# google/vizier

Hardware: NVIDIA H100
Metric: GP-UCB candidates scored/sec (higher is better)
Workload: dtype f64

## Files before the change

vizier_b200/csrc/async.cuh:

```cuda
#pragma once
#include <cuda.h>
#include <stdint.h>

namespace vzgp {

__device__ __forceinline__ void cp_async16(void* smem_dst, const void* gsrc, bool valid) {
  const unsigned s = static_cast<unsigned>(__cvta_generic_to_shared(smem_dst));
  const int sz = valid ? 16 : 0;
  asm volatile("cp.async.cg.shared.global [%0], [%1], 16, %2;\n" ::"r"(s), "l"(gsrc), "r"(sz) : "memory");
}
__device__ __forceinline__ void cp_async_commit() { asm volatile("cp.async.commit_group;\n" ::: "memory"); }
template <int N>
__device__ __forceinline__ void cp_async_wait() {
  asm volatile("cp.async.wait_group %0;\n" ::"n"(N) : "memory");
}
__device__ __forceinline__ unsigned smem_u32(const void* p) { return static_cast<unsigned>(__cvta_generic_to_shared(p)); }
__device__ __forceinline__ void mbar_init(uint64_t* bar, unsigned count) {
  asm volatile("mbarrier.init.shared::cta.b64 [%0], %1;\n" ::"r"(smem_u32(bar)), "r"(count) : "memory");
}
__device__ __forceinline__ void mbar_expect_tx(uint64_t* bar, unsigned bytes) {
  asm volatile("mbarrier.arrive.expect_tx.shared::cta.b64 _, [%0], %1;\n" ::"r"(smem_u32(bar)), "r"(bytes) : "memory");
}
__device__ __forceinline__ void mbar_wait(uint64_t* bar, unsigned parity) {
  unsigned ok;
  do {
    asm volatile(
        "{\n.reg .pred p;\nmbarrier.try_wait.parity.shared::cta.b64 p, [%1], %2;\nselp.u32 %0, 1, 0, p;\n}\n"
        : "=r"(ok)
        : "r"(smem_u32(bar)), "r"(parity)
        : "memory");
  } while (!ok);
}
__device__ __forceinline__ void tma_load_2d(void* smem_dst, const CUtensorMap* map, int c0, int c1, uint64_t* bar) {
  asm volatile(
      "cp.async.bulk.tensor.2d.shared::cluster.global.mbarrier::complete_tx::bytes [%0], [%1, {%2, %3}], [%4];\n" ::"r"(smem_u32(smem_dst)),
      "l"(reinterpret_cast<uint64_t>(map)), "r"(c0), "r"(c1), "r"(smem_u32(bar))
      : "memory");
}
__device__ __forceinline__ void fence_proxy_async() { asm volatile("fence.proxy.async;\n" ::: "memory"); }

__device__ __forceinline__ unsigned cluster_ctarank() {
  unsigned r;
  asm volatile("mov.u32 %0, %%cluster_ctarank;\n" : "=r"(r));
  return r;
}
__device__ __forceinline__ unsigned cluster_nctarank() {
  unsigned r;
  asm volatile("mov.u32 %0, %%cluster_nctarank;\n" : "=r"(r));
  return r;
}
__device__ __forceinline__ void cluster_sync() {
  asm volatile("barrier.cluster.arrive.release;\nbarrier.cluster.wait.acquire;\n" ::: "memory");
}
__device__ __forceinline__ void mbar_arrive_cluster(const uint64_t* bar, unsigned rank) {
  asm volatile(
      "{\n.reg .b32 ra;\nmapa.shared::cluster.u32 ra, %0, %1;\nmbarrier.arrive.shared::cluster.b64 _, [ra];\n}\n" ::"r"(
          smem_u32(bar)),
      "r"(rank)
      : "memory");
}
__device__ __forceinline__ void tma_load_2d_multicast(void* smem_dst, const CUtensorMap* map, int c0, int c1, uint64_t* bar,
                                                      uint16_t cta_mask) {
  asm volatile(
      "cp.async.bulk.tensor.2d.shared::cluster.global.mbarrier::complete_tx::bytes.multicast::cluster [%0], [%1, {%2, %3}], [%4], %5;\n" ::"r"(
          smem_u32(smem_dst)),
      "l"(reinterpret_cast<uint64_t>(map)), "r"(c0), "r"(c1), "r"(smem_u32(bar)), "h"(cta_mask)
      : "memory");
}


}
```

vizier_b200/csrc/score.cu:

```cuda
#include <cuda.h>

#include <climits>
#include <cstring>
#include <map>
#include <mutex>
#include <tuple>

#include "launchers.h"
#include "matern_fast.cuh"
#include "score_small.cuh"
#include "topk_merge.cuh"
#include "tiles.cuh"

namespace vzgp {

using GP1 = GemmCfg<64, 64, 16, 4, 4>;
constexpr int kThreads = 256;
constexpr int kBlockThreads = 288;
static_assert(GP1::kThreads == kThreads, "phase 1 maps one d2 block to every math thread");

constexpr int kBN = 128;
constexpr int kBK = 32;
constexpr int kStages = 4;
__host__ __device__ constexpr int pair_pos(int r) { return (((r >> 4) * 8 + (r & 7)) << 1) | ((r >> 3) & 1); }
__host__ __device__ constexpr int pair_row(int pos) { return ((pos >> 4) << 4) + ((pos >> 1) & 7) + ((pos & 1) << 3); }
static_assert(pair_row(pair_pos(13)) == 13 && pair_row(pair_pos(58)) == 58 && pair_pos(8) == 1, "pair order round trip");
constexpr int kABox = (kTM / 2) * 16;
constexpr int kBHalf = kBN * 16;
constexpr int kStageDoubles = 4 * kABox + 2 * kBHalf;
constexpr unsigned kStageBytes = kStageDoubles * sizeof(double);
constexpr int kCluster = 2;
constexpr int kBPieces = kCluster < 2 ? 2 : kCluster;
constexpr int kBPieceRows = 2 * kBN / kBPieces;
static_assert(kBPieces % 2 == 0 && kBN % (kBPieces / 2) == 0, "B pieces tile the two halves of a stage");

#ifdef VZ_SCORE_TIMING
constexpr int kScoreCounters = 11;
__device__ unsigned long long g_score_t[kScoreCounters];
#define VZ_ST(...) __VA_ARGS__
#else
#define VZ_ST(...)
#endif

template <bool WITH_LINF, bool GENERIC>
__global__ void __launch_bounds__(kBlockThreads, 1) k_score(const __grid_constant__ ScoreArgs a) {
  extern __shared__ double smem_raw[];
  double* smem = smem_raw + (((1024u - (static_cast<unsigned>(__cvta_generic_to_shared(smem_raw)) & 1023u)) & 1023u) >> 3);
  constexpr int LD = kLD1;
  const int dc = a.kp.dc, dk = a.kp.dk, np = a.np;
  double* ring = smem;
  double* sa = ring;
  double* sb = sa + dc * LD;
  double* s_alpha = ring + (kStages * kStageDoubles > 3 * kMaxDc * kLD1 ? kStages * kStageDoubles : 3 * kMaxDc * kLD1);
  double* s_mu = s_alpha + 128;
  double* s_linf = s_mu + 64;
  double* s_rowsq = s_linf + 64;
  uint64_t* full_bar = reinterpret_cast<uint64_t*>(s_rowsq + 256);
  uint64_t* empty_bar = full_bar + kStages;
  int32_t* za = reinterpret_cast<int32_t*>(full_bar + 8);
  int32_t* zb = za + dk * LD;
  uint8_t* s_mask = reinterpret_cast<uint8_t*>(zb + dk * LD);

  const int tid = threadIdx.x, lane = tid & 31, warp = tid >> 5;
  const int ty = tid / 16, tx = tid % 16;
  const int wm = warp & 1, wn = warp >> 1;
  const int fr = lane >> 2, fk = lane & 3;
  const int pr = ((fr & 1) << 2) | (fr >> 1);
  double* scr = a.scratch + (size_t)blockIdx.x * kTM * np;
  const unsigned crank = cluster_ctarank(), ncta = cluster_nctarank();
  auto tile_gate = [&]() { if (ncta > 1) cluster_sync(); else __syncthreads(); };
  if (tid < kMaxDc) s_mask[tid] = a.tr.mask[tid];
  if (tid == 0) {
    for (int s = 0; s < kStages; ++s) { mbar_init(full_bar + s, 1); mbar_init(empty_bar + s, ncta * (kThreads / 32)); }
    asm volatile("fence.mbarrier_init.release.cluster;\n" ::: "memory");
  }
  tile_gate();
  int clamped = 0;
  unsigned slab_n = 0;
  const bool is_producer = warp == kThreads / 32;
  auto consumer_sync = [&]() { asm volatile("bar.sync 1, %0;\n" ::"n"(kThreads) : "memory"); };
  VZ_ST(long long t_p1 = 0, t_gate = 0, t_p2 = 0, t_tile = 0, t_wait = 0, w_tile = 0, n_tiles = 0;)
  VZ_ST(long long t_d2 = 0, t_mat = 0, t_st = 0, t_sync = 0;)

  const int ntiles = (a.M + kTM - 1) / kTM;
  const int nblocks = (np + kBN - 1) / kBN;
  const int nsplit = a.nsplit;
  const double* XTs = a.XT;
  const double* XTu = a.XT + (size_t)dc * np;

  for (int w0 = blockIdx.x - crank; w0 < ntiles * nsplit; w0 += gridDim.x) {
    const int work = w0 + crank;
    const int tile = work / nsplit, split = work - tile * nsplit;
    const int m0 = tile * kTM;
    const int nq = (nsplit == 1) ? nblocks : ((split == nblocks - 1 - split) ? 1 : 2);
    auto block_of = [&](int q) { return (nsplit == 1) ? q : (q == 0 ? split : nblocks - 1 - split); };
    auto slabs_in = [&](int jb) { int kend = (jb + 1) * kBN; if (kend > np) kend = np; return kend / kBK; };
    if (is_producer) {
      tile_gate();
      VZ_ST(w_tile = 0;)
      if (lane == 0) {
        const uint16_t cmask = (uint16_t)((1u << ncta) - 1u);
        for (int q = 0; q < nq; ++q) {
          const int jb = block_of(q), nsl = slabs_in(jb);
          for (int ks = 0; ks < nsl; ++ks) {
            const int stage = slab_n % kStages;
            VZ_ST(const long long t0 = clock64();)
            mbar_wait(empty_bar + stage, ((slab_n / kStages) & 1) ^ 1);
            VZ_ST(w_tile += clock64() - t0;)
            double* base = ring + stage * kStageDoubles;
            const int k0 = ks * kBK;
            mbar_expect_tx(full_bar + stage, kStageBytes);
            for (int h = 0; h < 4; ++h)
              tma_load_2d(base + h * kABox, &a.mapA, 2 * k0 + 16 * h, (int)blockIdx.x * (kTM / 2), full_bar + stage);
            for (int p = (int)crank; p < kBPieces; p += (int)ncta) {
              const int half = p / (kBPieces / 2), r0 = (p % (kBPieces / 2)) * kBPieceRows;
              double* dst = base + 4 * kABox + half * kBHalf + r0 * 16;
              if (ncta > 1) tma_load_2d_multicast(dst, &a.mapB, k0 + 16 * half, jb * kBN + r0, full_bar + stage, cmask);
              else tma_load_2d(dst, &a.mapB, k0 + 16 * half, jb * kBN + r0, full_bar + stage);
            }
            ++slab_n;
          }
        }
      }
      __syncwarp();
      VZ_ST(if (m0 < a.M) t_wait += w_tile;)
      continue;
    }
    VZ_ST(const long long t_tile0 = clock64(); w_tile = 0;)
    consumer_sync();
    for (int e = tid; e < kTM * dc; e += kThreads) {
      const int r = e / dc, d = e - r * dc;
      const int gr = m0 + r;
      const double v = gr < a.M ? __ldg(a.Xs + (size_t)gr * dc + d) : 0.0;
      sa[d * LD + pair_pos(r)] = WITH_LINF ? v : v * a.kp.inv_ls_c[d];
    }
    if (dk > 0) stage_rows_T_i32(a.Zs, a.M, dk, m0, kTM, za, LD, kThreads);

    auto stage_trials = [&](int jb, int buf) {
      double* dst = sb + buf * dc * LD;
      const double* src = WITH_LINF ? XTu : XTs;
      for (int c = tid; c < dc * 32; c += kThreads) {
        const int d = c >> 5, q = c & 31;
        cp_async16(dst + d * LD + q * 2, src + (size_t)d * np + jb * 64 + q * 2, true);
      }
      if (tid < 32) cp_async16(s_alpha + buf * 64 + tid * 2, a.alpha + jb * 64 + tid * 2, true);
    };
    double mu_part[4], lmin[4];
#pragma unroll
    for (int i = 0; i < 4; ++i) { mu_part[i] = 0.0; lmin[i] = INFINITY; }
    const int nj = np / 64;
    stage_trials(0, 0);
    cp_async_commit();
    for (int jb = 0; jb < nj; ++jb) {
      VZ_ST(long long tc = clock64();)
      const int buf = jb & 1;
      if (jb + 1 < nj) stage_trials(jb + 1, buf ^ 1);
      cp_async_commit();
      cp_async_wait<1>();
      consumer_sync();
      if (dk > 0) {
        stage_rows_T_i32(a.Z, np, dk, jb * 64, 64, zb, LD, kThreads);
        consumer_sync();
      }
      VZ_ST(t_sync += clock64() - tc; tc = clock64();)
      const double* sbj = sb + buf * dc * LD;
      const double* alj = s_alpha + buf * 64;
      double d2[4][4], lf[4][4];
#pragma unroll
      for (int i = 0; i < 4; ++i)
#pragma unroll
        for (int j = 0; j < 4; ++j) { d2[i][j] = 0.0; lf[i][j] = 0.0; }
      for (int d = 0; d < dc; ++d) {
        const double2 a0 = *reinterpret_cast<const double2*>(sa + d * LD + GP1::row_of(ty, 0));
        const double2 a1 = *reinterpret_cast<const double2*>(sa + d * LD + GP1::row_of(ty, 2));
        const double2 b0 = *reinterpret_cast<const double2*>(sbj + d * LD + GP1::col_of(tx, 0));
        const double2 b1 = *reinterpret_cast<const double2*>(sbj + d * LD + GP1::col_of(tx, 2));
        const double aa[4] = {a0.x, a0.y, a1.x, a1.y}, bb[4] = {b0.x, b0.y, b1.x, b1.y};
        if (WITH_LINF) {
          const double w = a.kp.inv_ls2_c[d];
          const bool in_tr = s_mask[d] != 0;
#pragma unroll
          for (int i = 0; i < 4; ++i)
#pragma unroll
            for (int j = 0; j < 4; ++j) {
              const double df = aa[i] - bb[j];
              d2[i][j] = fma(df * df, w, d2[i][j]);
              if (in_tr) lf[i][j] = fmax(lf[i][j], fabs(df));
            }
        } else {
#pragma unroll
          for (int i = 0; i < 4; ++i)
#pragma unroll
            for (int j = 0; j < 4; ++j) {
              const double df = aa[i] - bb[j];
              d2[i][j] = fma(df, df, d2[i][j]);
            }
        }
      }
      for (int k = 0; k < dk; ++k) {
        const double w = a.kp.inv_ls2_k[k];
#pragma unroll
        for (int i = 0; i < 4; ++i) {
          const int avz = za[k * LD + pair_row(GP1::row_of(ty, i))];
#pragma unroll
          for (int j = 0; j < 4; ++j) d2[i][j] += (avz != zb[k * LD + GP1::col_of(tx, j)]) ? w : 0.0;
        }
      }
      VZ_ST(t_d2 += clock64() - tc; tc = clock64();)
      if (WITH_LINF) {
#pragma unroll
        for (int i = 0; i < 4; ++i)
#pragma unroll
          for (int j = 0; j < 4; ++j)
            if ((jb * 64 + GP1::col_of(tx, j)) < a.tr.rows) lmin[i] = fmin(lmin[i], lf[i][j]);
      }
      double kv[4][4];
#pragma unroll
      for (int i = 0; i < 4; ++i)
#pragma unroll
        for (int j = 0; j < 4; ++j) kv[i][j] = matern52_fast(d2[i][j], a.kp.sf2);
#pragma unroll
      for (int i = 0; i < 4; ++i)
#pragma unroll
        for (int j = 0; j < 4; ++j) {
          const int cj = GP1::col_of(tx, j);
          kv[i][j] = (jb * 64 + cj) < a.n_valid ? kv[i][j] : 0.0;
          mu_part[i] = fma(kv[i][j], alj[cj], mu_part[i]);
        }
      VZ_ST(t_mat += clock64() - tc; tc = clock64();)
#pragma unroll
      for (int ip = 0; ip < 2; ++ip) {
        double* dst = scr + (size_t)(GP1::row_of(ty, 2 * ip) >> 1) * (2 * np) + 2 * jb * 64;
#pragma unroll
        for (int j = 0; j < 4; ++j)
          *reinterpret_cast<double2*>(dst + 2 * GP1::col_of(tx, j)) = make_double2(kv[2 * ip][j], kv[2 * ip + 1][j]);
      }
      VZ_ST(t_st += clock64() - tc;)
      VZ_ST(tc = clock64();)
      consumer_sync();
      VZ_ST(t_sync += clock64() - tc;)
    }
    cp_async_wait<0>();
#pragma unroll
    for (int i = 0; i < 4; ++i) {
#pragma unroll
      for (int o = 8; o > 0; o >>= 1) {
        mu_part[i] += __shfl_xor_sync(0xffffffffu, mu_part[i], o);
        if (WITH_LINF) lmin[i] = fmin(lmin[i], __shfl_xor_sync(0xffffffffu, lmin[i], o));
      }
      if (tx == 0) {
        s_mu[pair_row(GP1::row_of(ty, i))] = mu_part[i];
        s_linf[pair_row(GP1::row_of(ty, i))] = lmin[i];
      }
    }
    fence_proxy_async();
    VZ_ST(const long long t1 = clock64();)
    tile_gate();
    VZ_ST(const long long t2 = clock64();)

    double rowsq[2][2] = {{0.0, 0.0}, {0.0, 0.0}};
    for (int q = 0; q < nq; ++q) {
      const int jb = block_of(q);
      double acc[2][2][4][2];
#pragma unroll
      for (int mf = 0; mf < 2; ++mf)
#pragma unroll
        for (int f = 0; f < 2; ++f)
#pragma unroll
          for (int g = 0; g < 4; ++g) { acc[mf][f][g][0] = 0.0; acc[mf][f][g][1] = 0.0; }
      const int nsl = slabs_in(jb);
      const int col_base = jb * kBN + wn * 32;
      for (int ks = 0; ks < nsl; ++ks) {
        const int stage = slab_n % kStages;
        VZ_ST(const long long tw = clock64();)
        mbar_wait(full_bar + stage, (slab_n / kStages) & 1);
        VZ_ST(w_tile += clock64() - tw;)
        ++slab_n;
        const double* stg = ring + stage * kStageDoubles;
        const double* Arow0 = stg + (wm * 16 + fr) * 16;
        const double* Brow0 = stg + 4 * kABox + (wn * 32 + pr) * 16;
        const int k0 = ks * kBK;
        auto group = [&](int h, bool diag) {
          const int co = ((((h & 1) * 4 + fk) ^ pr) * 2);
          auto live = [&](int g) { return !(diag && g < h); };
          double2 b[4];
#pragma unroll
          for (int g = 0; g < 4; ++g)
            if (live(g)) b[g] = *reinterpret_cast<const double2*>(Brow0 + (h >> 1) * kBHalf + g * 8 * 16 + co);
#pragma unroll
          for (int mf = 0; mf < 2; ++mf) {
            const double* Ah = Arow0 + h * kABox + mf * 8 * 16;
            const double2 a01 = *reinterpret_cast<const double2*>(Ah + (((2 * fk) ^ fr) * 2));
            const double2 a23 = *reinterpret_cast<const double2*>(Ah + (((2 * fk + 1) ^ fr) * 2));
#pragma unroll
            for (int g = 0; g < 4; ++g)
              if (live(g))
                dmma_16x8x8(acc[mf][0][g][0], acc[mf][0][g][1], acc[mf][1][g][0], acc[mf][1][g][1],
                            a01.x, a01.y, a23.x, a23.y, b[g].x, b[g].y);
          }
        };
        if (k0 < col_base) {
#pragma unroll 1
          for (int h = 0; h < 4; ++h) group(h, false);
        } else if (k0 == col_base) {
#pragma unroll 1
          for (int h = 0; h < 4; ++h) group(h, true);
        }
        __syncwarp();
        if ((unsigned)lane < ncta) mbar_arrive_cluster(empty_bar + stage, lane);
      }
#pragma unroll
      for (int mf = 0; mf < 2; ++mf)
#pragma unroll
        for (int f = 0; f < 2; ++f)
#pragma unroll
          for (int g = 0; g < 4; ++g) {
            rowsq[mf][f] = fma(acc[mf][f][g][0], acc[mf][f][g][0], rowsq[mf][f]);
            rowsq[mf][f] = fma(acc[mf][f][g][1], acc[mf][f][g][1], rowsq[mf][f]);
          }
    }
    VZ_ST(const long long t3 = clock64();)
    cp_async_wait<0>();
#pragma unroll
    for (int mf = 0; mf < 2; ++mf)
#pragma unroll
      for (int f = 0; f < 2; ++f) {
        rowsq[mf][f] += __shfl_xor_sync(0xffffffffu, rowsq[mf][f], 1);
        rowsq[mf][f] += __shfl_xor_sync(0xffffffffu, rowsq[mf][f], 2);
        if (fk == 0) s_rowsq[wn * 64 + wm * 32 + mf * 16 + f * 8 + fr] = rowsq[mf][f];
      }
    consumer_sync();
    if (tid < kTM) {
      const int r = tid, m = m0 + r;
      if (m < a.M) {
        const double rs = (s_rowsq[r] + s_rowsq[64 + r]) + (s_rowsq[128 + r] + s_rowsq[192 + r]);
        if (nsplit == 1) {
          emit_score<GENERIC>(a, m, rs, s_mu[r], s_linf[r], clamped);
        } else {
          a.part[(size_t)split * a.mpad + m] = rs;
          if (split == 0) {
            a.part[(size_t)nsplit * a.mpad + m] = s_mu[r];
            a.part[(size_t)(nsplit + 1) * a.mpad + m] = s_linf[r];
          }
        }
      }
    }
    VZ_ST(if (m0 < a.M) { t_p1 += t1 - t_tile0; t_gate += t2 - t1; t_p2 += t3 - t2; t_tile += clock64() - t_tile0; t_wait += w_tile; ++n_tiles; })
  }
  if (clamped) atomicAdd(a.clamp_count, clamped);
#ifdef VZ_SCORE_TIMING
  if (lane == 0) {
    if (is_producer) {
      atomicAdd(&g_score_t[6], (unsigned long long)t_wait);
    } else {
      atomicAdd(&g_score_t[5], (unsigned long long)t_wait);
      if (warp == 0) {
        atomicAdd(&g_score_t[0], (unsigned long long)n_tiles);
        atomicAdd(&g_score_t[1], (unsigned long long)t_p1);
        atomicAdd(&g_score_t[2], (unsigned long long)t_p2);
        atomicAdd(&g_score_t[3], (unsigned long long)t_gate);
        atomicAdd(&g_score_t[4], (unsigned long long)t_tile);
        atomicAdd(&g_score_t[7], (unsigned long long)t_d2);
        atomicAdd(&g_score_t[8], (unsigned long long)t_mat);
        atomicAdd(&g_score_t[9], (unsigned long long)t_st);
        atomicAdd(&g_score_t[10], (unsigned long long)t_sync);
      }
    }
  }
#endif
  if (ncta > 1) cluster_sync();
}

__global__ void k_score_finalize(const ScoreArgs a) {
  const int m = blockIdx.x * blockDim.x + threadIdx.x;
  int clamped = 0;
  if (m < a.M) {
    double rs = 0.0;
    for (int s = 0; s < a.nsplit; ++s) rs += a.part[(size_t)s * a.mpad + m];
    emit_score(a, m, rs, a.part[(size_t)a.nsplit * a.mpad + m], a.part[(size_t)(a.nsplit + 1) * a.mpad + m], clamped);
  }
  if (clamped) atomicAdd(a.clamp_count, clamped);
}

template <bool WITH_LINF>
__global__ void __launch_bounds__(kSmallThreads) k_cross_small(const ScoreArgs a) {
  extern __shared__ double smem_raw[];
  cross_small_block<WITH_LINF>(a, blockIdx.x, blockIdx.y >> 2, blockIdx.y & 3, smem_raw);
}
__global__ void __launch_bounds__(kSmallThreads) k_var_small(const __grid_constant__ ScoreArgs a) {
  extern __shared__ double smem_raw[];
  var_small_dispatch(a, blockIdx.x, blockIdx.y, smem_raw);
}
template <bool WITH_LINF>
__global__ void __launch_bounds__(256) k_small_finalize(const ScoreArgs a) {
  const int m = blockIdx.x * 32 + (threadIdx.x >> 3);
  int clamped = 0;
  small_finalize_8<WITH_LINF>(a, m, threadIdx.x & 7, m < a.M, clamped);
  if (clamped) atomicAdd(a.clamp_count, clamped);
}

size_t cross_small_smem_bytes(int dc, int dk) { return sizeof(double) * 2 * dc * kLD1 + sizeof(int32_t) * 2 * dk * kLD1; }
size_t var_small_smem_bytes() {
  const size_t cp = sizeof(double) * kVarStages * kVarStageDoubles, tma = 1024 + sizeof(double) * kVarStages * kVarTmaStageDoubles;
  return cp > tma ? cp : tma;
}

typedef CUresult (*EncodeTiledFn)(CUtensorMap*, CUtensorMapDataType, cuuint32_t, void*, const cuuint64_t*,
                                  const cuuint64_t*, const cuuint32_t*, const cuuint32_t*, CUtensorMapInterleave,
                                  CUtensorMapSwizzle, CUtensorMapL2promotion, CUtensorMapFloatOOBfill);

static EncodeTiledFn encode_tiled_fn() {
  static const EncodeTiledFn fn = [] {
    void* p = nullptr;
    cudaDriverEntryPointQueryResult qres;
    EncodeTiledFn f = nullptr;
    if (cudaGetDriverEntryPoint("cuTensorMapEncodeTiled", &p, cudaEnableDefault, &qres) == cudaSuccess &&
        qres == cudaDriverEntryPointSuccess)
      f = reinterpret_cast<EncodeTiledFn>(p);
    cudaGetLastError();
    return f;
  }();
  return fn;
}

static int make_map(CUtensorMap* m, const double* base, uint64_t rows, uint64_t cols, uint64_t ld, uint32_t box_rows,
                    bool l2_promotion = true) {
  EncodeTiledFn fn = encode_tiled_fn();
  if (!fn) { set_error("cuTensorMapEncodeTiled is not available from this driver"); return VZGP_ERR_CUDA; }
  cuuint64_t gdim[2] = {cols, rows};
  cuuint64_t gstride[1] = {ld * sizeof(double)};
  cuuint32_t box[2] = {16, box_rows};
  cuuint32_t estr[2] = {1, 1};
  CUresult r = fn(m, CU_TENSOR_MAP_DATA_TYPE_FLOAT64, 2, const_cast<double*>(base), gdim, gstride, box, estr,
                  CU_TENSOR_MAP_INTERLEAVE_NONE, CU_TENSOR_MAP_SWIZZLE_128B,
                  l2_promotion ? CU_TENSOR_MAP_L2_PROMOTION_L2_256B : CU_TENSOR_MAP_L2_PROMOTION_NONE,
                  CU_TENSOR_MAP_FLOAT_OOB_FILL_NONE);
  if (r != CUDA_SUCCESS) { set_error("cuTensorMapEncodeTiled failed with CUresult %d", (int)r); return VZGP_ERR_CUDA; }
  return 0;
}

int make_tensor_map_f64(void* map, const double* base, uint64_t rows, uint64_t cols, uint64_t ld, uint32_t box_rows) {
  static const bool promo = [] { const char* e = getenv("VZGP_DF_L2PROMO"); return e && e[0] == '1'; }();
  return make_map(static_cast<CUtensorMap*>(map), base, rows, cols, ld, box_rows, promo);
}

int make_tensor_map_u8(void* map, const void* base, int rank, const uint64_t* dims, const uint64_t* strides,
                       const uint32_t* box, bool promote_256) {
  EncodeTiledFn fn = encode_tiled_fn();
  if (!fn) { set_error("cuTensorMapEncodeTiled is not available from this driver"); return VZGP_ERR_CUDA; }
  cuuint64_t gdim[3], gstride[2];
  cuuint32_t bx[3], estr[3] = {1, 1, 1};
  for (int i = 0; i < rank; ++i) { gdim[i] = dims[i]; bx[i] = box[i]; }
  for (int i = 0; i + 1 < rank; ++i) gstride[i] = strides[i];
  CUresult r = fn(static_cast<CUtensorMap*>(map), CU_TENSOR_MAP_DATA_TYPE_UINT8, (cuuint32_t)rank, const_cast<void*>(base),
                  gdim, gstride, bx, estr, CU_TENSOR_MAP_INTERLEAVE_NONE, CU_TENSOR_MAP_SWIZZLE_128B,
                  promote_256 ? CU_TENSOR_MAP_L2_PROMOTION_L2_256B : CU_TENSOR_MAP_L2_PROMOTION_L2_128B,
                  CU_TENSOR_MAP_FLOAT_OOB_FILL_NONE);
  if (r != CUDA_SUCCESS) { set_error("cuTensorMapEncodeTiled (u8) failed with CUresult %d", (int)r); return VZGP_ERR_CUDA; }
  return 0;
}

size_t score_smem_bytes(int dc, int dk, bool with_linf) {
  (void)with_linf; (void)dc;
  const size_t big = kStages * kStageDoubles > 3 * kMaxDc * kLD1 ? kStages * kStageDoubles : 3 * kMaxDc * kLD1;
  return 1024 + sizeof(double) * (big + 128 + 64 * 2 + 256 + 8) +
         sizeof(int32_t) * dk * 2 * kLD1 + kMaxDc;
}

static int ensure_scratch(vzgp_handle* h, size_t scratch_bytes) {
  if (scratch_bytes > h->scratch.bytes || h->scratch_window != h->scratch.ptr) {
    VZ_TRY(h->scratch.reserve(scratch_bytes));
    cudaDeviceProp prop;
    if (cudaGetDeviceProperties(&prop, h->device) == cudaSuccess && prop.persistingL2CacheMaxSize > 0) {
      size_t want = h->scratch.bytes;
      if (want > (size_t)prop.persistingL2CacheMaxSize) want = (size_t)prop.persistingL2CacheMaxSize;
      cudaDeviceSetLimit(cudaLimitPersistingL2CacheSize, want);
      cudaStreamAttrValue attr;
      memset(&attr, 0, sizeof(attr));
      size_t win = h->scratch.bytes;
      if (win > (size_t)prop.accessPolicyMaxWindowSize) win = (size_t)prop.accessPolicyMaxWindowSize;
      attr.accessPolicyWindow.base_ptr = h->scratch.ptr;
      attr.accessPolicyWindow.num_bytes = win;
      attr.accessPolicyWindow.hitRatio = win > 0 ? (float)((double)want / (double)win > 1.0 ? 1.0 : (double)want / (double)win) : 0.f;
      attr.accessPolicyWindow.hitProp = cudaAccessPropertyPersisting;
      attr.accessPolicyWindow.missProp = cudaAccessPropertyStreaming;
      cudaStreamSetAttribute(h->stream, cudaStreamAttributeAccessPolicyWindow, &attr);
      cudaGetLastError();
    }
    h->scratch_window = h->scratch.ptr;
  }
  return 0;
}

static int max_active_clusters(const void* kfn, const cudaLaunchConfig_t& cfg, int* out) {
  static std::mutex mu;
  static std::map<std::tuple<int, const void*, size_t>, int> cache;
  int dev = 0;
  VZ_CUDA(cudaGetDevice(&dev));
  std::lock_guard<std::mutex> lock(mu);
  int& n = cache[{dev, kfn, cfg.dynamicSmemBytes}];
  if (n == 0) {
    cudaLaunchConfig_t c = cfg;
    c.gridDim = dim3(cfg.attrs[0].val.clusterDim.x);
    VZ_CUDA(cudaOccupancyMaxActiveClusters(&n, kfn, &c));
    if (n <= 0) { set_error("no cluster of the score kernel fits on device %d", dev); return VZGP_ERR_CUDA; }
  }
  *out = n;
  return 0;
}

void fill_score_args(vzgp_handle* h, const double* Xs, const int32_t* Zs, int M, const vzgp_acq* acq, const AcqFn* fn,
                     double* score, double* mu, double* sigma, double* linf, ScoreArgs* pa) {
  ScoreArgs& a = *pa;
  const int ntiles = (M + kTM - 1) / kTM;
  a.Xs = Xs; a.Zs = Zs; a.M = M;
  a.XT = h->XT.as<double>(); a.Z = h->Z.as<int32_t>();
  a.np = h->np; a.n_valid = h->n_valid;
  a.Linv = h->Linv.as<double>(); a.ldi = h->np;
  a.alpha = h->alpha.as<double>();
  a.kp = h->kp; a.sn2 = h->sn2;
  a.acq = acq_fn_of(acq, fn);
  a.tr = trust_region_of(h, *acq, acq->tr_strict);
  a.scratch = h->scratch.as<double>();
  a.mpad = ntiles * kTM;
  a.nsplit = 1;
  a.box_rows = kTM;
  static const int tma_small = [] { const char* e = getenv("VZGP_SMALL_TMA"); return e ? atoi(e) : 1; }();
  a.use_tma = tma_small;
  a.part = a.part_rs = a.part_mu = a.part_linf = nullptr;
  a.score = score; a.mu = mu; a.sigma = sigma; a.linf = linf;
  a.clamp_count = h->small.as<int>();
}

int prepare_small_score(vzgp_handle* h, const double* Xs, const int32_t* Zs, int M, const vzgp_acq* acq,
                        double* score, double* mu, double* sigma, double* linf, ScoreArgs* a, bool* with_linf,
                        const AcqFn* fn) {
  const int ntiles = (M + kTM - 1) / kTM;
  VZ_TRY(ensure_scratch(h, (size_t)ntiles * kTM * h->np * sizeof(double)));
  fill_score_args(h, Xs, Zs, M, acq, fn, score, mu, sigma, linf, a);
  const int nvb = h->np / kVarCols, nmb = h->np / 64;
  VZ_TRY(h->Tws.reserve(sizeof(double) * (size_t)(nvb + 2 * nmb) * a->mpad));
  a->part_rs = h->Tws.as<double>();
  a->part_mu = a->part_rs + (size_t)nvb * a->mpad;
  a->part_linf = a->part_mu + (size_t)nmb * a->mpad;
  *with_linf = (linf != nullptr) || tr_needs_distance(a->tr);
  a->box_rows = ntiles == 1 ? ((M + 7) / 8) * 8 : kTM;
  VZ_TRY(make_map(&a->mapA, a->scratch, (uint64_t)ntiles * kTM, (uint64_t)h->np, (uint64_t)h->np, (uint32_t)a->box_rows));
  VZ_TRY(make_map(&a->mapB, a->Linv, (uint64_t)h->np, (uint64_t)h->np, (uint64_t)h->np, kVarCols));
  return 0;
}

struct GeneralArgs {
  const double* Xs;
  const double* Ks;
  const double* W;
  const double* X;
  const double* alpha;
  int mc, np, n_valid, dc;
  KernelParams kp;
  double sn2, mean_const;
  AcqFn acq;
  TrustRegion tr;
  int want_linf;
  double* score; double* mu; double* sigma; double* linf;
  int* clamp_count;
};

__global__ void __launch_bounds__(256) k_general_finalize(GeneralArgs a) {
  const int m = blockIdx.x * (blockDim.x / 32) + threadIdx.x / 32, lane = threadIdx.x & 31;
  if (m >= a.mc) return;
  const double* ks = a.Ks + (size_t)m * a.np;
  const double* w = a.W + (size_t)m * a.np;
  double mean = 0.0, rs = 0.0;
  for (int j = lane; j < a.n_valid; j += 32) mean = fma(ks[j], a.alpha[j], mean);
  for (int j = lane; j < a.np; j += 32) rs = fma(w[j], w[j], rs);
  double dist = a.want_linf ? tr_lane_distance(a.tr, a.Xs + (size_t)m * a.dc, a.X, a.dc, lane) : INFINITY;
#pragma unroll
  for (int o = 16; o > 0; o >>= 1) {
    mean += __shfl_xor_sync(0xffffffffu, mean, o);
    rs += __shfl_xor_sync(0xffffffffu, rs, o);
    dist = fmin(dist, __shfl_xor_sync(0xffffffffu, dist, o));
  }
  if (lane != 0) return;
  double kss = a.kp.sf2;
  if (a.kp.use_linear) {
    double uu = 0.0;
    for (int d = 0; d < a.dc; ++d) {
      const double u = fma(a.Xs[(size_t)m * a.dc + d], a.kp.inv_ls_c[d], -a.kp.lin_b);
      uu = fma(u, u, uu);
    }
    kss = fma(a.kp.lin_a, uu, kss);
  }
  mean += a.mean_const;
  double var = kss - rs + a.sn2;
  if (var < 0.0) { var = 0.0; atomicAdd(a.clamp_count, 1); }
  const double sd = sqrt(var);
  a.score[m] = tr_apply(a.tr, acq_value(a.acq, mean, sd), dist);
  if (a.mu) a.mu[m] = mean;
  if (a.sigma) a.sigma[m] = sd;
  if (a.linf) a.linf[m] = dist;
}

int general_chunk_buffers(vzgp_handle* h, GeneralChunk* c) {
  const int np = h->np, dc = h->dc, dk = h->dk;
  const size_t nks = (size_t)kGeneralChunk * np, nx = (size_t)kGeneralChunk * (dc > 0 ? dc : 1);
  VZ_TRY(h->gen.reserve(sizeof(double) * (2 * nks + nx) + sizeof(int32_t) * (size_t)kGeneralChunk * (dk > 0 ? dk : 1)));
  c->Ks = h->gen.as<double>();
  c->W = c->Ks + nks;
  c->Xp = c->W + nks;
  c->Zp = reinterpret_cast<int32_t*>(c->Xp + nx);
  return 0;
}

int launch_general_chunk(vzgp_handle* h, const double* Xs, const int32_t* Zs, int mc, const GeneralChunk& c) {
  const int np = h->np, dc = h->dc, dk = h->dk, mp = round_up(mc, 64);
  if (dc > 0) VZ_TRY(launch_pad_rows(h, Xs, mc, dc, mp, c.Xp));
  if (dk > 0) VZ_TRY(launch_pad_rows_i32(h, Zs, mc, dk, mp, c.Zp));
  VZ_TRY(launch_cross_kernel(h, c.Xp, c.Zp, mp, h->X.as<double>(), h->Z.as<int32_t>(), np, h->n_valid, h->kp, c.Ks, np));
  return launch_gemm_nt_tri(h, c.Ks, np, mp, h->Linv.as<double>(), np, np, c.W, np);
}

static int launch_score_general(vzgp_handle* h, const double* Xs, const int32_t* Zs, int M, const vzgp_acq* acq,
                                const AcqFn* fn, double* score, double* mu, double* sigma, double* linf) {
  const int np = h->np, dc = h->dc, dk = h->dk;
  constexpr int kChunk = kGeneralChunk;
  GeneralChunk c;
  VZ_TRY(general_chunk_buffers(h, &c));
  GeneralArgs a;
  a.Ks = c.Ks; a.W = c.W; a.Xs = c.Xp; a.X = h->X.as<double>(); a.alpha = h->alpha.as<double>();
  a.np = np; a.n_valid = h->n_valid; a.dc = dc; a.kp = h->kp; a.sn2 = h->sn2; a.mean_const = h->mean_const;
  a.acq = acq_fn_of(acq, fn);
  a.tr = trust_region_of(h, *acq, acq->tr_strict);
  a.want_linf = (linf != nullptr) || tr_needs_distance(a.tr);
  a.clamp_count = h->small.as<int>();
  for (int m0 = 0; m0 < M; m0 += kChunk) {
    const int mc = M - m0 < kChunk ? M - m0 : kChunk;
    VZ_TRY(launch_general_chunk(h, dc > 0 ? Xs + (size_t)m0 * dc : Xs, dk > 0 ? Zs + (size_t)m0 * dk : Zs, mc, c));
    a.mc = mc;
    a.score = score + m0; a.mu = mu ? mu + m0 : nullptr; a.sigma = sigma ? sigma + m0 : nullptr;
    a.linf = linf ? linf + m0 : nullptr;
    k_general_finalize<<<(mc + 7) / 8, 256, 0, h->stream>>>(a);
    VZ_CHECK_LAUNCH();
    h->launches++;
  }
  return 0;
}

int launch_score(vzgp_handle* h, const double* Xs, const int32_t* Zs, int M, const vzgp_acq* acq,
                 double* score, double* mu, double* sigma, double* linf, const AcqFn* fn) {
  if (M <= 0) return 0;
  auto record = [&](int route, int nsplit, int grid) { h->score_route = route; h->score_nsplit = nsplit; h->score_grid = grid; };
  if (h->kp.use_linear) {
    record(VZGP_ROUTE_GENERAL, 0, 0);
    return launch_score_general(h, Xs, Zs, M, acq, fn, score, mu, sigma, linf);
  }
  const int ntiles = (M + kTM - 1) / kTM;
  const int nblocks = (h->np + kBN - 1) / kBN;
  static const int env_small_tiles = [] {
    const char* e = getenv("VZGP_SMALL_TILES");
    return e ? atoi(e) : 8;
  }();
  const int small_tiles_max = h->small_tiles >= 0 ? h->small_tiles : env_small_tiles;
  ScoreArgs a;
  if (ntiles <= small_tiles_max) {
    record(VZGP_ROUTE_SMALL, 0, 0);
    bool with_linf = false;
    VZ_TRY(prepare_small_score(h, Xs, Zs, M, acq, score, mu, sigma, linf, &a, &with_linf, fn));
    const int nvb = h->np / kVarCols, nmb = h->np / 64;
    const size_t sm1 = cross_small_smem_bytes(h->dc, h->dk), sm2 = var_small_smem_bytes();
    const dim3 g1(nmb, ntiles * 4), g2(nvb, ntiles);
    if (with_linf) {
      VZ_TRY(raise_dyn_smem((const void*)k_cross_small<true>, sm1));
      k_cross_small<true><<<g1, kSmallThreads, sm1, h->stream>>>(a);
    } else {
      VZ_TRY(raise_dyn_smem((const void*)k_cross_small<false>, sm1));
      k_cross_small<false><<<g1, kSmallThreads, sm1, h->stream>>>(a);
    }
    VZ_CHECK_LAUNCH();
    VZ_TRY(raise_dyn_smem((const void*)k_var_small, sm2));
    k_var_small<<<g2, kSmallThreads, sm2, h->stream>>>(a);
    VZ_CHECK_LAUNCH();
    if (with_linf) k_small_finalize<true><<<(M + 31) / 32, 256, 0, h->stream>>>(a);
    else k_small_finalize<false><<<(M + 31) / 32, 256, 0, h->stream>>>(a);
    VZ_CHECK_LAUNCH();
    h->launches += 3;
    return 0;
  }
  {
    static const int env_i8 = [] { const char* e = getenv("VZGP_SCORE_I8"); return e ? atoi(e) : 0; }();
    const int want = h->score_i8 >= 0 ? h->score_i8 : env_i8;
    if (want && score_i8_eligible(h, M)) {
      record(VZGP_ROUTE_I8, 1, 0);
      return launch_score_i8(h, Xs, Zs, M, acq, score, mu, sigma, linf, fn);
    }
  }
  int nsplit = 1;
  if (ntiles * 2 <= h->sm_count && nblocks >= 2) nsplit = (nblocks + 1) / 2;
  const int nwork = ntiles * nsplit;
  const int csize = nsplit == 1 ? kCluster : 1;
  const bool need_linf = (linf != nullptr) || tr_needs_distance(trust_region_of(h, *acq, acq->tr_strict));
  const size_t sm = score_smem_bytes(h->dc, h->dk, need_linf);
  if (sm > 227 * 1024) {
    set_error("score kernel needs %zu bytes of shared memory (Dc=%d with trust-region distance)", sm, h->dc);
    return VZGP_ERR_UNSUPPORTED;
  }
  const bool generic = !acq_fn_is_ucb(acq_fn_of(acq, fn));
  const void* kfn = generic ? (need_linf ? (const void*)k_score<true, true> : (const void*)k_score<false, true>)
                            : (need_linf ? (const void*)k_score<true, false> : (const void*)k_score<false, false>);
  VZ_TRY(raise_dyn_smem(kfn, sm));
  cudaLaunchAttribute cattr[1];
  cattr[0].id = cudaLaunchAttributeClusterDimension;
  cattr[0].val.clusterDim.x = csize; cattr[0].val.clusterDim.y = 1; cattr[0].val.clusterDim.z = 1;
  cudaLaunchConfig_t cfg = {};
  cfg.blockDim = dim3(kBlockThreads); cfg.dynamicSmemBytes = sm; cfg.stream = h->stream;
  cfg.attrs = cattr; cfg.numAttrs = 1;
  int slots = h->sm_count;
  if (csize > 1) VZ_TRY(max_active_clusters(kfn, cfg, &slots));
  const int want = (nwork + csize - 1) / csize;
  const int grid = (want < slots ? want : slots) * csize;
  cfg.gridDim = dim3(grid);
  record(nsplit > 1 ? VZGP_ROUTE_SPLIT : VZGP_ROUTE_CLUSTER, nsplit, grid);
  VZ_TRY(ensure_scratch(h, (size_t)grid * kTM * h->np * sizeof(double)));
  fill_score_args(h, Xs, Zs, M, acq, fn, score, mu, sigma, linf, &a);
  VZ_TRY(make_map(&a.mapA, a.scratch, (uint64_t)grid * (kTM / 2), 2 * (uint64_t)h->np, 2 * (uint64_t)h->np, kTM / 2));
  static_assert(4 * kABox == kTM * kBK, "four A boxes hold one slab of K*");
  VZ_TRY(make_map(&a.mapB, a.Linv, (uint64_t)h->np, (uint64_t)h->np, (uint64_t)h->np, kBPieceRows));
  a.nsplit = nsplit;
  if (nsplit > 1) {
    VZ_TRY(h->Tws.reserve(sizeof(double) * (size_t)(nsplit + 2) * a.mpad));
    a.part = h->Tws.as<double>();
  }
  void* kargs[] = {&a};
  VZ_CUDA(cudaLaunchKernelExC(&cfg, kfn, kargs));
  VZ_CHECK_LAUNCH();
  h->launches++;
  if (nsplit > 1) {
    k_score_finalize<<<(M + 255) / 256, 256, 0, h->stream>>>(a);
    VZ_CHECK_LAUNCH();
    h->launches++;
  }
  return 0;
}

struct PeCombine {
  int mode;
  double ucb, explore, penalty, threshold;
  TrustRegion tr;
};
__global__ void k_pe_combine(int M, PeCombine p, const double* __restrict__ mu, const double* __restrict__ sd,
                             const double* __restrict__ sd_all, const double* __restrict__ linf,
                             double* __restrict__ score) {
  const int m = blockIdx.x * blockDim.x + threadIdx.x;
  if (m >= M) return;
  double acq;
  if (p.mode == 0) {
    acq = fma(p.ucb, sd_all[m], mu[m]);
  } else {
    const double explore_ucb = fma(sd[m], p.explore, mu[m]);
    acq = sd_all[m] + p.penalty * fmin(explore_ucb - p.threshold, 0.0);
  }
  score[m] = tr_apply(p.tr, acq, linf[m]);
}

int launch_score_pe(vzgp_handle* hA, vzgp_handle* hB, const double* Xs, const int32_t* Zs, int M,
                    const vzgp_pe_params* pe, double* score, double* mu, double* sigma, double* sigma_all) {
  if (M <= 0) return 0;
  VZ_TRY(hA->pe_tmp.reserve(sizeof(double) * 6 * (size_t)M));
  double* t = hA->pe_tmp.as<double>();
  double* mu_a = mu ? mu : t;
  double* sd_a = sigma ? sigma : t + M;
  double* sd_b = sigma_all ? sigma_all : t + 2 * (size_t)M;
  double* linf_b = t + 3 * (size_t)M;
  double* dummy_a = t + 4 * (size_t)M;
  double* dummy_b = t + 5 * (size_t)M;
  const vzgp_acq none = posterior_request(), accb = posterior_request(pe->tr_dim_mask, pe->tr_rows);
  PeCombine p;
  p.mode = pe->mode; p.ucb = pe->ucb_coefficient; p.explore = pe->explore_coefficient;
  p.penalty = pe->penalty_coefficient; p.threshold = pe->threshold;
  p.tr = trust_region_of(hB, *pe, true);
  VZ_TRY(launch_score(hA, Xs, Zs, M, &none, dummy_a, mu_a, sd_a, nullptr));
  VZ_TRY(launch_score(hB, Xs, Zs, M, &accb, dummy_b, nullptr, sd_b, tr_needs_distance(p.tr) ? linf_b : nullptr));
  k_pe_combine<<<(M + 255) / 256, 256, 0, hA->stream>>>(M, p, mu_a, sd_a, sd_b, linf_b, score);
  VZ_CHECK_LAUNCH();
  hA->launches++;
  return 0;
}

struct StackCombine {
  int E;
  double alpha[16];
  AcqFn acq;
  TrustRegion tr;
};
__global__ void k_stack_combine(int M, StackCombine p, const double* __restrict__ mu_e, const double* __restrict__ sd_e,
                                const double* __restrict__ linf, double* __restrict__ score, double* __restrict__ mu,
                                double* __restrict__ sigma) {
  const int m = blockIdx.x * blockDim.x + threadIdx.x;
  if (m >= M) return;
  double mean = mu_e[m], sd = sd_e[m];
  for (int e = 1; e < p.E; ++e) {
    mean += mu_e[(size_t)e * M + m];
    sd = pow(sd_e[(size_t)e * M + m], p.alpha[e]) * pow(sd, 1.0 - p.alpha[e]);
  }
  score[m] = tr_apply(p.tr, acq_value(p.acq, mean, sd), linf[m]);
  if (mu) mu[m] = mean;
  if (sigma) sigma[m] = sd;
}

int launch_score_stack(vzgp_handle* const* hs, int E, const double* alphas, const double* Xs, const int32_t* Zs, int M,
                       const vzgp_acq* acq, double* score, double* mu, double* sigma, double* linf, const AcqFn* fn) {
  if (M <= 0) return 0;
  vzgp_handle* top = hs[E - 1];
  VZ_TRY(top->pe_tmp.reserve(sizeof(double) * (2 * (size_t)E + 2) * (size_t)M));
  double* t = top->pe_tmp.as<double>();
  double* mu_e = t;
  double* sd_e = t + (size_t)E * M;
  double* linf_buf = linf ? linf : t + 2 * (size_t)E * M;
  double* dummy = t + (2 * (size_t)E + 1) * M;
  StackCombine p;
  p.E = E; p.acq = acq_fn_of(acq, fn);
  p.tr = trust_region_of(top, *acq, acq->tr_strict);
  const bool want_linf = tr_needs_distance(p.tr) || linf != nullptr;
  const vzgp_acq none = posterior_request(acq->tr_dim_mask, acq->tr_rows);
  for (int e = 0; e < E; ++e)
    VZ_TRY(launch_score(hs[e], Xs, Zs, M, &none, dummy, mu_e + (size_t)e * M, sd_e + (size_t)e * M,
                        (e == E - 1 && want_linf) ? linf_buf : nullptr));
  for (int e = 0; e < 16; ++e) p.alpha[e] = e < E ? alphas[e] : 0.0;
  k_stack_combine<<<(M + 255) / 256, 256, 0, top->stream>>>(M, p, mu_e, sd_e, linf_buf, score, mu, sigma);
  VZ_CHECK_LAUNCH();
  top->launches++;
  return 0;
}

__global__ void __launch_bounds__(32) k_set_pe_combine(int n_sets, int q, PeCombine p, const double* __restrict__ cov, int ldc,
                                                       const double* __restrict__ mu_a, const double* __restrict__ sd_a,
                                                       const double* __restrict__ linf, double* __restrict__ score,
                                                       double* __restrict__ sd_all) {
  __shared__ double c[16][17];
  const int s = blockIdx.x, lane = threadIdx.x;
  if (s >= n_sets) return;
  const int r0 = s * q;
  for (int e = lane; e < q * q; e += 32) c[e / q][e % q] = cov[(size_t)(r0 + e / q) * ldc + r0 + e % q];
  __syncwarp();
  if (sd_all && lane < q) sd_all[r0 + lane] = sqrt(fmax(c[lane][lane], 0.0));
  double logdet = 0.0;
  bool bad = false;
  for (int k = 0; k < q; ++k) {
    const double d = c[k][k];
    if (!(d > 0.0) || !isfinite(d)) { bad = true; break; }
    logdet += log(d);
    __syncwarp();
    const double inv = 1.0 / d;
    for (int i = k + 1 + lane; i < q; i += 32) {
      const double lik = c[i][k] * inv;
      for (int j = k + 1; j <= i; ++j) c[i][j] -= lik * c[j][k];
    }
    __syncwarp();
  }
  double pen = 0.0, tr = 0.0;
  for (int i = lane; i < q; i += 32) {
    pen += fmin(mu_a[r0 + i] + p.explore * sd_a[r0 + i] - p.threshold, 0.0);
    if (p.tr.apply) tr += tr_set_term(p.tr, linf[r0 + i]);
  }
#pragma unroll
  for (int o = 16; o > 0; o >>= 1) {
    pen += __shfl_xor_sync(0xffffffffu, pen, o);
    tr += __shfl_xor_sync(0xffffffffu, tr, o);
  }
  if (lane == 0) score[s] = (bad ? -INFINITY : logdet) + p.penalty * pen + tr;
}

int launch_set_pe_combine(vzgp_handle* h, int n_sets, int q, const vzgp_pe_params* pe, const double* cov, int ldc,
                          const double* mu_a, const double* sd_a, const double* linf, double* score, double* sd_all) {
  PeCombine p;
  p.mode = 1; p.ucb = pe->ucb_coefficient; p.explore = pe->explore_coefficient;
  p.penalty = pe->penalty_coefficient; p.threshold = pe->threshold;
  p.tr = trust_region_of(h, *pe, true);
// ... 208 lines not shown
```

Baseline: 34.68 million.

## Stage K* tiles in shared memory and write scratch via TMA bulk stores

Phase 1 now writes the K* block into swizzled shared-memory staging buffers, and a single thread issues TMA tensor stores to a re-laid-out scratch (box-major, 16-wide rows). Phase 2's TMA loads are changed to match. The aim is to replace scattered per-thread global stores with asynchronous bulk stores that overlap with the next block's compute. The change also adds triple-buffered trial staging with alpha stored inline, software-prefetches the d-loop operands, and disables the L2 persisting window on the cluster route. In exchange it carries more complex smem accounting that depends on dc, extra bulk-group waits, and shares the smem ring between the phases.

```diff
diff --git a/vizier_b200/csrc/async.cuh b/vizier_b200/csrc/async.cuh
--- a/vizier_b200/csrc/async.cuh
+++ b/vizier_b200/csrc/async.cuh
@@ -37,7 +37,23 @@
       "l"(reinterpret_cast<uint64_t>(map)), "r"(c0), "r"(c1), "r"(smem_u32(bar))
       : "memory");
 }
+__device__ __forceinline__ void tma_store_2d(const CUtensorMap* map, int c0, int c1, const void* smem_src) {
+  asm volatile("cp.async.bulk.tensor.2d.global.shared::cta.bulk_group [%0, {%1, %2}], [%3];\n" ::"l"(
+                   reinterpret_cast<uint64_t>(map)),
+               "r"(c0), "r"(c1), "r"(smem_u32(smem_src))
+               : "memory");
+}
+__device__ __forceinline__ void bulk_commit() { asm volatile("cp.async.bulk.commit_group;\n" ::: "memory"); }
+template <int N>
+__device__ __forceinline__ void bulk_wait_read() {
+  asm volatile("cp.async.bulk.wait_group.read %0;\n" ::"n"(N) : "memory");
+}
+template <int N>
+__device__ __forceinline__ void bulk_wait() {
+  asm volatile("cp.async.bulk.wait_group %0;\n" ::"n"(N) : "memory");
+}
 __device__ __forceinline__ void fence_proxy_async() { asm volatile("fence.proxy.async;\n" ::: "memory"); }
+__device__ __forceinline__ void fence_proxy_async_smem() { asm volatile("fence.proxy.async.shared::cta;\n" ::: "memory"); }
 
 __device__ __forceinline__ unsigned cluster_ctarank() {
   unsigned r;
diff --git a/vizier_b200/csrc/score.cu b/vizier_b200/csrc/score.cu
--- a/vizier_b200/csrc/score.cu
+++ b/vizier_b200/csrc/score.cu
@@ -33,6 +33,16 @@
 constexpr int kBPieces = kCluster < 2 ? 2 : kCluster;
 constexpr int kBPieceRows = 2 * kBN / kBPieces;
 static_assert(kBPieces % 2 == 0 && kBN % (kBPieces / 2) == 0, "B pieces tile the two halves of a stage");
+constexpr int kStgDoubles = 8 * kABox;
+constexpr int kTrialBufs = 3;
+__host__ __device__ constexpr int trial_stride(int dc) { return dc * kLD1 + 64; }
+__host__ __device__ constexpr int phase1_doubles(int dc, int nstg) { return nstg * kStgDoubles + dc * kLD1 + kTrialBufs * trial_stride(dc); }
+__host__ __device__ constexpr int stg_buffers(int dc) {
+  return phase1_doubles(dc, 3) <= kStages * kStageDoubles ? 3 : phase1_doubles(dc, 2) <= kStages * kStageDoubles ? 2 : 1;
+}
+static_assert(phase1_doubles(kMaxDc, 1) <= kStages * kStageDoubles, "phase-1 staging fits in the ring at every dc");
+static_assert(stg_buffers(45) == 3 && stg_buffers(46) == 2 && stg_buffers(61) == 2 && stg_buffers(62) == 1,
+              "the staging plan switches at dc = 46 and 62 (tested on both sides)");
 
 #ifdef VZ_SCORE_TIMING
 constexpr int kScoreCounters = 11;
@@ -49,10 +59,11 @@
   constexpr int LD = kLD1;
   const int dc = a.kp.dc, dk = a.kp.dk, np = a.np;
   double* ring = smem;
-  double* sa = ring;
+  const int nstg = stg_buffers(dc);
+  double* sk = ring;
+  double* sa = sk + nstg * kStgDoubles;
   double* sb = sa + dc * LD;
-  double* s_alpha = ring + (kStages * kStageDoubles > 3 * kMaxDc * kLD1 ? kStages * kStageDoubles : 3 * kMaxDc * kLD1);
-  double* s_mu = s_alpha + 128;
+  double* s_mu = ring + kStages * kStageDoubles;
   double* s_linf = s_mu + 64;
   double* s_rowsq = s_linf + 64;
   uint64_t* full_bar = reinterpret_cast<uint64_t*>(s_rowsq + 256);
@@ -66,7 +77,7 @@
   const int wm = warp & 1, wn = warp >> 1;
   const int fr = lane >> 2, fk = lane & 3;
   const int pr = ((fr & 1) << 2) | (fr >> 1);
-  double* scr = a.scratch + (size_t)blockIdx.x * kTM * np;
+  auto scratch_box_row = [&](int g) { return ((int)blockIdx.x * (np / 8) + g) * (kTM / 2); };
   const unsigned crank = cluster_ctarank(), ncta = cluster_nctarank();
   auto tile_gate = [&]() { if (ncta > 1) cluster_sync(); else __syncthreads(); };
   if (tid < kMaxDc) s_mask[tid] = a.tr.mask[tid];
@@ -111,7 +122,7 @@
             const int k0 = ks * kBK;
             mbar_expect_tx(full_bar + stage, kStageBytes);
             for (int h = 0; h < 4; ++h)
-              tma_load_2d(base + h * kABox, &a.mapA, 2 * k0 + 16 * h, (int)blockIdx.x * (kTM / 2), full_bar + stage);
+              tma_load_2d(base + h * kABox, &a.mapA, 0, scratch_box_row(k0 / 8 + h), full_bar + stage);
             for (int p = (int)crank; p < kBPieces; p += (int)ncta) {
               const int half = p / (kBPieces / 2), r0 = (p % (kBPieces / 2)) * kBPieceRows;
               double* dst = base + 4 * kABox + half * kBHalf + r0 * 16;
@@ -137,13 +148,19 @@
     if (dk > 0) stage_rows_T_i32(a.Zs, a.M, dk, m0, kTM, za, LD, kThreads);
 
     auto stage_trials = [&](int jb, int buf) {
-      double* dst = sb + buf * dc * LD;
+      double* dst = sb + buf * trial_stride(dc);
       const double* src = WITH_LINF ? XTu : XTs;
       for (int c = tid; c < dc * 32; c += kThreads) {
         const int d = c >> 5, q = c & 31;
         cp_async16(dst + d * LD + q * 2, src + (size_t)d * np + jb * 64 + q * 2, true);
       }
-      if (tid < 32) cp_async16(s_alpha + buf * 64 + tid * 2, a.alpha + jb * 64 + tid * 2, true);
+      if (tid < 32) cp_async16(dst + dc * LD + tid * 2, a.alpha + jb * 64 + tid * 2, true);
+    };
+    auto store_step = [&](int jb) {
+      const double* src = sk + (jb % nstg) * kStgDoubles;
+#pragma unroll 1
+      for (int h = 0; h < 8; ++h) tma_store_2d(&a.mapA, 0, scratch_box_row(8 * jb + h), src + h * kABox);
+      bulk_commit();
     };
     double mu_part[4], lmin[4];
 #pragma unroll
@@ -153,32 +170,42 @@
     cp_async_commit();
     for (int jb = 0; jb < nj; ++jb) {
       VZ_ST(long long tc = clock64();)
-      const int buf = jb & 1;
-      if (jb + 1 < nj) stage_trials(jb + 1, buf ^ 1);
+      const int buf = jb % kTrialBufs;
+      if (jb + 1 < nj) stage_trials(jb + 1, (jb + 1) % kTrialBufs);
       cp_async_commit();
       cp_async_wait<1>();
+      if (tid == 0) { if (nstg == 3) bulk_wait_read<1>(); else bulk_wait_read<0>(); }
       consumer_sync();
       if (dk > 0) {
         stage_rows_T_i32(a.Z, np, dk, jb * 64, 64, zb, LD, kThreads);
         consumer_sync();
       }
       VZ_ST(t_sync += clock64() - tc; tc = clock64();)
-      const double* sbj = sb + buf * dc * LD;
-      const double* alj = s_alpha + buf * 64;
+      if (jb > 0 && tid == 0) store_step(jb - 1);
+      VZ_ST(t_st += clock64() - tc; tc = clock64();)
+      const double* sbj = sb + buf * trial_stride(dc);
+      const double* alj = sbj + dc * LD;
       double d2[4][4], lf[4][4];
 #pragma unroll
       for (int i = 0; i < 4; ++i)
 #pragma unroll
         for (int j = 0; j < 4; ++j) { d2[i][j] = 0.0; lf[i][j] = 0.0; }
+      auto ld2 = [](const double* p) { return *reinterpret_cast<const double2*>(p); };
+      double2 a0 = ld2(sa + GP1::row_of(ty, 0)), a1 = ld2(sa + GP1::row_of(ty, 2));
+      double2 b0 = ld2(sbj + GP1::col_of(tx, 0)), b1 = ld2(sbj + GP1::col_of(tx, 2));
+      double w_n = WITH_LINF ? a.kp.inv_ls2_c[0] : 0.0;
+      bool in_tr_n = WITH_LINF ? s_mask[0] != 0 : false;
       for (int d = 0; d < dc; ++d) {
-        const double2 a0 = *reinterpret_cast<const double2*>(sa + d * LD + GP1::row_of(ty, 0));
-        const double2 a1 = *reinterpret_cast<const double2*>(sa + d * LD + GP1::row_of(ty, 2));
-        const double2 b0 = *reinterpret_cast<const double2*>(sbj + d * LD + GP1::col_of(tx, 0));
-        const double2 b1 = *reinterpret_cast<const double2*>(sbj + d * LD + GP1::col_of(tx, 2));
+        const int dn = d + 1 < dc ? d + 1 : d;
+        const double2 a0n = ld2(sa + dn * LD + GP1::row_of(ty, 0)), a1n = ld2(sa + dn * LD + GP1::row_of(ty, 2));
+        const double2 b0n = ld2(sbj + dn * LD + GP1::col_of(tx, 0)), b1n = ld2(sbj + dn * LD + GP1::col_of(tx, 2));
         const double aa[4] = {a0.x, a0.y, a1.x, a1.y}, bb[4] = {b0.x, b0.y, b1.x, b1.y};
+        a0 = a0n; a1 = a1n; b0 = b0n; b1 = b1n;
         if (WITH_LINF) {
-          const double w = a.kp.inv_ls2_c[d];
-          const bool in_tr = s_mask[d] != 0;
+          const double w = w_n;
+          const bool in_tr = in_tr_n;
+          w_n = a.kp.inv_ls2_c[dn];
+          in_tr_n = s_mask[dn] != 0;
 #pragma unroll
           for (int i = 0; i < 4; ++i)
 #pragma unroll
@@ -228,18 +255,36 @@
           mu_part[i] = fma(kv[i][j], alj[cj], mu_part[i]);
         }
       VZ_ST(t_mat += clock64() - tc; tc = clock64();)
-#pragma unroll
-      for (int ip = 0; ip < 2; ++ip) {
-        double* dst = scr + (size_t)(GP1::row_of(ty, 2 * ip) >> 1) * (2 * np) + 2 * jb * 64;
-#pragma unroll
-        for (int j = 0; j < 4; ++j)
-          *reinterpret_cast<double2*>(dst + 2 * GP1::col_of(tx, j)) = make_double2(kv[2 * ip][j], kv[2 * ip + 1][j]);
-      }
+      if (nstg == 1) {
+        if (tid == 0) bulk_wait_read<0>();
+        consumer_sync();
+      }
+      VZ_ST(t_sync += clock64() - tc; tc = clock64();)
+      {
+        double* stg = sk + (jb % nstg) * kStgDoubles;
+        const bool swap = (tx & 4) != 0;
+#pragma unroll
+        for (int ip = 0; ip < 2; ++ip) {
+          const int p = 16 * ip + ty;
+#pragma unroll
+          for (int jj = 0; jj < 4; ++jj) {
+            const int j = jj ^ 1;
+            const double v0 = swap ? kv[2 * ip][j] : kv[2 * ip][jj], v1 = swap ? kv[2 * ip + 1][j] : kv[2 * ip + 1][jj];
+            const int cj = GP1::col_of(tx, jj) ^ (swap ? 1 : 0);
+            *reinterpret_cast<double2*>(stg + (cj >> 3) * kABox + p * 16 + (((cj & 7) ^ (p & 7)) * 2)) = make_double2(v0, v1);
+          }
+        }
+      }
+      fence_proxy_async_smem();
       VZ_ST(t_st += clock64() - tc;)
-      VZ_ST(tc = clock64();)
-      consumer_sync();
-      VZ_ST(t_sync += clock64() - tc;)
-    }
+    }
+    VZ_ST(long long tc = clock64();)
+    consumer_sync();
+    VZ_ST(t_sync += clock64() - tc; tc = clock64();)
+    if (tid == 0) store_step(nj - 1);
+    VZ_ST(t_st += clock64() - tc; tc = clock64();)
+    if (tid == 0) bulk_wait<0>();
+    VZ_ST(t_sync += clock64() - tc;)
     cp_async_wait<0>();
 #pragma unroll
     for (int i = 0; i < 4; ++i) {
@@ -462,14 +507,23 @@
 
 size_t score_smem_bytes(int dc, int dk, bool with_linf) {
   (void)with_linf; (void)dc;
-  const size_t big = kStages * kStageDoubles > 3 * kMaxDc * kLD1 ? kStages * kStageDoubles : 3 * kMaxDc * kLD1;
-  return 1024 + sizeof(double) * (big + 128 + 64 * 2 + 256 + 8) +
+  return 1024 + sizeof(double) * (kStages * kStageDoubles + 64 * 2 + 256 + 8) +
          sizeof(int32_t) * dk * 2 * kLD1 + kMaxDc;
 }
 
-static int ensure_scratch(vzgp_handle* h, size_t scratch_bytes) {
-  if (scratch_bytes > h->scratch.bytes || h->scratch_window != h->scratch.ptr) {
-    VZ_TRY(h->scratch.reserve(scratch_bytes));
+static int ensure_scratch(vzgp_handle* h, size_t scratch_bytes, bool persist) {
+  if (scratch_bytes > h->scratch.bytes) VZ_TRY(h->scratch.reserve(scratch_bytes));
+  if (!persist) {
+    if (h->scratch_window != nullptr) {
+      cudaStreamAttrValue attr;
+      memset(&attr, 0, sizeof(attr));
+      cudaStreamSetAttribute(h->stream, cudaStreamAttributeAccessPolicyWindow, &attr);
+      cudaGetLastError();
+      h->scratch_window = nullptr;
+    }
+    return 0;
+  }
+  if (h->scratch_window != h->scratch.ptr) {
     cudaDeviceProp prop;
     if (cudaGetDeviceProperties(&prop, h->device) == cudaSuccess && prop.persistingL2CacheMaxSize > 0) {
       size_t want = h->scratch.bytes;
@@ -536,7 +590,7 @@
                         double* score, double* mu, double* sigma, double* linf, ScoreArgs* a, bool* with_linf,
                         const AcqFn* fn) {
   const int ntiles = (M + kTM - 1) / kTM;
-  VZ_TRY(ensure_scratch(h, (size_t)ntiles * kTM * h->np * sizeof(double)));
+  VZ_TRY(ensure_scratch(h, (size_t)ntiles * kTM * h->np * sizeof(double), true));
   fill_score_args(h, Xs, Zs, M, acq, fn, score, mu, sigma, linf, a);
   const int nvb = h->np / kVarCols, nmb = h->np / 64;
   VZ_TRY(h->Tws.reserve(sizeof(double) * (size_t)(nvb + 2 * nmb) * a->mpad));
@@ -720,9 +774,9 @@
   const int grid = (want < slots ? want : slots) * csize;
   cfg.gridDim = dim3(grid);
   record(nsplit > 1 ? VZGP_ROUTE_SPLIT : VZGP_ROUTE_CLUSTER, nsplit, grid);
-  VZ_TRY(ensure_scratch(h, (size_t)grid * kTM * h->np * sizeof(double)));
+  VZ_TRY(ensure_scratch(h, (size_t)grid * kTM * h->np * sizeof(double), false));
   fill_score_args(h, Xs, Zs, M, acq, fn, score, mu, sigma, linf, &a);
-  VZ_TRY(make_map(&a.mapA, a.scratch, (uint64_t)grid * (kTM / 2), 2 * (uint64_t)h->np, 2 * (uint64_t)h->np, kTM / 2));
+  VZ_TRY(make_map(&a.mapA, a.scratch, (uint64_t)grid * (kTM / 2) * (h->np / 8), 16, 16, kTM / 2));
   static_assert(4 * kABox == kTM * kBK, "four A boxes hold one slab of K*");
   VZ_TRY(make_map(&a.mapB, a.Linv, (uint64_t)h->np, (uint64_t)h->np, (uint64_t)h->np, kBPieceRows));
   a.nsplit = nsplit;
```

Result: faster. 36.15 million (median of 6 runs) (+4.3%).
